# rubychen0611/image-analogies-python

Hardware: AMD Instinct MI355X
Metric: B' pixels/sec (brute-force match, 5-level pyramid) + MFMA util @1/2/4/8 GPU (higher is better)
Workload: dtype f16 rotated split (R16 MFMA screen: 3 principal components as f16 pairs, 52 as f16, f32 accumulate) + f64 (rotation, exact rescore, pyramids); 1 GPU; c4: A/A' 2048x2048 x B 1024x1024, 5-level, DB sharded, brute force; levels_cap=5, jobs_per_gpu=1, streams_per_gpu=1, jobs_per_launch=1, parallelism=single

## Files before the change

image-analogies-python_amd/csrc/ia_exact.h:

```cpp
#pragma once
#include "ia_imgwin.h"
#include "ia_split16.h"

#include <float.h>

namespace ia {

constexpr int TILE_H8 = DB16_GROUPS * 64;

__device__ __forceinline__ void best_update(double &bd, long long &bi, double d, long long i) {
    if (d < bd || (d == bd && i < bi)) { bd = d; bi = i; }
}

__device__ __forceinline__ void rescore_thresholds(float emin, float amax0, double nqq,
                                                   double &Tseg, double &Trow, bool &force_full) {
    constexpr double U32 = 5.9604644775390625e-08;
    const double A = (double)amax0;
    const double eps = 70.0 * U32 * (2.0 * A * sqrt(nqq) + A * A);
    const Split16Db sc = split16_db_scale(amax0);
    const int eq = split16_q_scale(nqq, sc.R);
    const int e2 = sc.ea + eq;
    const double em = ldexp((double)emin, -e2);
    const double eps16 = U32 * (300.0 * A * sqrt(nqq) + 50.0 * A * A);
    const double slack = 1e-12 * (fabs(em) + nqq + A * A);
    Tseg = ldexp(em + 2.0 * eps16 + slack, e2);
    Trow = ldexp(em + eps16 + eps + slack, sc.ea);
    force_full = eq + sc.R < -10;
}

__device__ __forceinline__ void load_row16(const half8 *__restrict__ db16, long r,
                                           half8 (&g0)[DB16_GROUPS], half8 (&g1)[DB16_GROUPS]) {
    const half8 *t = db16 + (r >> 5) * TILE_H8 + (r & 31);
#pragma unroll
    for (int g = 0; g < DB16_GROUPS; ++g) {
        g0[g] = t[g * 64];
        g1[g] = t[g * 64 + 32];
    }
}

__device__ __forceinline__ float rescreen16(const half8 (&g0)[DB16_GROUPS],
                                            const half8 (&g1)[DB16_GROUPS], const float *qf,
                                            float twoR) {
    float acc = 0.f;
#pragma unroll
    for (int k = 0; k < IA_DP; ++k) {
        _Float16 hi, lo;
        if (k < 24) { hi = g0[k >> 3][k & 7]; lo = g0[4 + (k >> 3)][k & 7]; }
        else if (k < 32) { hi = g0[3][k & 7]; lo = g1[3][k & 7]; }
        else { hi = g1[(k - 32) >> 3][k & 7]; lo = g1[4 + ((k - 32) >> 3)][k & 7]; }
        const float x = (float)hi + (float)lo;
        acc = fmaf(x, k < 55 ? qf[(k & 1) * 28 + (k >> 1)] : twoR, acc);
    }
    return acc;
}

__device__ __forceinline__ float win_x(const char *bf, const char *bc, int k) {
    const uint32_t v = *reinterpret_cast<const uint32_t *>(((k < 55 && win_coarse(k)) ? bc : bf) + win_off(k));
    return (float)__builtin_bit_cast(_Float16, (uint16_t)(v & 0xffffu)) +
           (float)__builtin_bit_cast(_Float16, (uint16_t)(v >> 16));
}
__device__ __forceinline__ void win_terms2(const char *r0, const char *r1, const float *qf, int k,
                                           float &a0, float &a1) {
    const uint32_t v0 = *reinterpret_cast<const uint32_t *>(r0);
    const uint32_t v1 = *reinterpret_cast<const uint32_t *>(r1);
    const float f = qf[(k & 1) * 28 + (k >> 1)];
    a0 = fmaf((float)__builtin_bit_cast(_Float16, (uint16_t)(v0 & 0xffffu)) +
              (float)__builtin_bit_cast(_Float16, (uint16_t)(v0 >> 16)), f, a0);
    a1 = fmaf((float)__builtin_bit_cast(_Float16, (uint16_t)(v1 & 0xffffu)) +
              (float)__builtin_bit_cast(_Float16, (uint16_t)(v1 >> 16)), f, a1);
}
__device__ __forceinline__ void rescreen_win2(const char *wb, int p, const float *qf, float twoR,
                                              float &e0, float &e1) {
    const char *bf0 = wb + 4 * p, *bc0 = wb + 4 * (p >> 1);
    const char *bf1 = bf0 + 256, *bc1 = bc0 + 128;
    float a0 = 0.f, a1 = 0.f;
    int k = 0;
#pragma unroll 1
    for (int r = 0; r < 3; ++r) {
        const int o = WB_FINE + r * WC_PC * 16 + 12;
#pragma unroll
        for (int c = 0; c < 3; ++c, ++k) win_terms2(bc0 + o + 4 * c, bc1 + o + 4 * c, qf, k, a0, a1);
    }
#pragma unroll 1
    for (int r = 0; r < 5; ++r) {
        const int o = r * WF_PC * 16 + 8;
#pragma unroll
        for (int c = 0; c < 5; ++c, ++k) win_terms2(bf0 + o + 4 * c, bf1 + o + 4 * c, qf, k, a0, a1);
    }
#pragma unroll 1
    for (int r = 3; r < 6; ++r) {
        const int o = WB_FINE + r * WC_PC * 16 + 12;
#pragma unroll
        for (int c = 0; c < 3; ++c, ++k) win_terms2(bc0 + o + 4 * c, bc1 + o + 4 * c, qf, k, a0, a1);
    }
#pragma unroll 1
    for (int r = 5; r < 8; ++r) {
        const int o = r * WF_PC * 16 + 8;
        const int nc = r < 7 ? 5 : 2;
#pragma unroll
        for (int c = 0; c < 5; ++c, ++k)
            if (c < nc) win_terms2(bf0 + o + 4 * c, bf1 + o + 4 * c, qf, k, a0, a1);
    }
    const uint32_t v0 = *reinterpret_cast<const uint32_t *>(bf0 + WB_FINE + WB_COARSE);
    const uint32_t v1 = *reinterpret_cast<const uint32_t *>(bf1 + WB_FINE + WB_COARSE);
    a0 = fmaf((float)__builtin_bit_cast(_Float16, (uint16_t)(v0 & 0xffffu)) +
              (float)__builtin_bit_cast(_Float16, (uint16_t)(v0 >> 16)), twoR, a0);
    a1 = fmaf((float)__builtin_bit_cast(_Float16, (uint16_t)(v1 & 0xffffu)) +
              (float)__builtin_bit_cast(_Float16, (uint16_t)(v1 >> 16)), twoR, a1);
    e0 = a0;
    e1 = a1;
}
static_assert(win_off(0) == WB_FINE + 12 && win_off(9) == 8 && win_off(34) == WB_FINE + 3 * WC_PC * 16 + 12 &&
                  win_off(43) == 5 * WF_PC * 16 + 8 && win_off(54) == 7 * WF_PC * 16 + 12 &&
                  win_off(55) == WB_FINE + WB_COARSE,
              "rescreen_win2 walks win_off's rows");

constexpr int WIN_PPL = (WIN_PIECES + 63) / 64;
typedef unsigned int piece_t __attribute__((ext_vector_type(4)));
__device__ __forceinline__ void win_load(const ImgDb &im, long lrow, int lane, piece_t (&pc)[WIN_PPL]) {
    const WinSrc ws = win_src(im, lrow);
#pragma unroll
    for (int j = 0; j < WIN_PPL; ++j) {
        const int i = lane + 64 * j;
        if (i < WIN_PIECES) pc[j] = *reinterpret_cast<const piece_t *>(win_piece(im, ws, i));
    }
}
constexpr int WIN_SLOT = WIN_PPL * 1024;
__device__ __forceinline__ void win_dma(const ImgDb &im, long lrow, int lane, char *wb) {
    asm volatile("" : "+v"(lane));
    const WinSrc ws = win_src(im, lrow);
#pragma unroll
    for (int j = 0; j < WIN_PPL; ++j) {
        const int i = lane + 64 * j;
        __builtin_amdgcn_global_load_lds((const void *)win_piece(im, ws, i < WIN_PIECES ? i : 0),
                                         (void *)(wb + j * 1024), 16, 0, 0);
    }
}
__device__ __forceinline__ void win_dma_wait() {
    asm volatile("s_waitcnt vmcnt(0)" ::: "memory");
    __builtin_amdgcn_wave_barrier();
}
__device__ __forceinline__ void win_store(char *wb, int lane, const piece_t (&pc)[WIN_PPL]) {
#pragma unroll
    for (int j = 0; j < WIN_PPL; ++j) {
        const int i = lane + 64 * j;
        if (i < WIN_PIECES) reinterpret_cast<piece_t *>(wb)[i] = pc[j];
    }
}
__device__ __forceinline__ void wave_lds_sync() {
    __builtin_amdgcn_fence(__ATOMIC_RELEASE, "wavefront");
    __builtin_amdgcn_wave_barrier();
    __builtin_amdgcn_fence(__ATOMIC_ACQUIRE, "wavefront");
}

constexpr int RESCORE_SEGCAP = 1024;
constexpr int RESCORE_REG = 8;
constexpr int RESCORE_RPT = 2;
constexpr int RESCORE_ROWCAP = 512;
static_assert(DB_SEG_MAX <= RESCORE_RPT * 256, "one re-screen step per segment");

__device__ __forceinline__ int vidx(int i) {
    asm volatile("" : "+v"(i));
    return i;
}

__device__ __forceinline__ void segmin_load(const float4 *sq4, long n4, float4 (&v)[RESCORE_REG]) {
    const int tid = threadIdx.x;
    const long lim = tid < 256 ? n4 : 0;
#pragma unroll
    for (int j = 0; j < RESCORE_REG; ++j) {
        const long i = tid + (long)j * 256;
        const float4 x = sq4[i < n4 ? i : 0];
        v[j] = i < lim ? x : make_float4(FLT_MAX, FLT_MAX, FLT_MAX, FLT_MAX);
    }
}
__device__ __forceinline__ float segmin_wave_min(const float4 *sq4, long n4, const float4 (&v)[RESCORE_REG]) {
    const int tid = threadIdx.x;
    const long lim = tid < 256 ? n4 : 0;
    float emin = FLT_MAX;
#pragma unroll
// ... 96 lines not shown
```

image-analogies-python_amd/csrc/ia_rot16.h:

```cpp
#pragma once
#include "ia_internal.h"
#include "ia_split16.h"

namespace ia {

#ifndef IA_R16_P
#define IA_R16_P 3
#endif
constexpr int R16_P = IA_R16_P;
constexpr int R16_NL = 2 * R16_P;
constexpr int R16_M0 = R16_NL + 1;
constexpr int R16_NH = R16_M0 + IA_D;
constexpr int R16_SLOTS = (R16_NH + 16) / 16 * 16;
constexpr int R16_MFMA = R16_SLOTS / 16;
constexpr int R16_TILE_H8 = R16_MFMA * 64;
constexpr int R16_ROW_B = R16_SLOTS * 2;
constexpr int R16_LD = 56;
constexpr int R16_ROT_FLOATS = 13 * 256;
constexpr int R16_ROT_B = R16_ROT_FLOATS * 4;

static inline size_t r16_askseg_off(long nrows) { return (size_t)db_rows_padded(nrows) * R16_ROW_B; }
static inline size_t r16_askc_off(long nrows) {
    return r16_askseg_off(nrows) + img_align((size_t)db_nsegs(nrows) * 4);
}
static inline const unsigned char *r16_askc(const void *dbr, long nrows) {
    return reinterpret_cast<const unsigned char *>(dbr) + r16_askc_off(nrows);
}
static_assert(R16_LD * R16_LD <= R16_ROT_FLOATS, "rotation buffer");

__host__ __device__ constexpr int r16_qpos(int s) {
    return (((s & 15) >> 3) * R16_MFMA + (s >> 4)) * 8 + (s & 7);
}
__host__ __device__ constexpr int r16_dgrp(int s, int j) { return (s >> 4) * 64 + ((s & 15) >> 3) * 32 + j; }

#ifndef IA_R16_SHAPE
#define IA_R16_SHAPE 16
#endif
constexpr bool R16_S16 = IA_R16_SHAPE == 16 && R16_MFMA == 4;
constexpr double R16_EPS_A2 = R16_S16 ? 90.0 : 60.0;
__device__ __forceinline__ double r16_eps(double A, double nqq, double Askip, double nsk) {
    constexpr double U32 = 5.9604644775390625e-08;
    return U32 * (360.0 * A * sqrt(nqq) + R16_EPS_A2 * A * A) + 0x1p-9 * 1.01 * Askip * sqrt(nsk);
}

__device__ __forceinline__ void r16_thresholds(float emin, float amax0, float askip, double nqq, double nsk,
                                               double &Tseg, bool &force_full) {
    const double A = (double)amax0;
    const Split16Db sc = split16_db_scale(amax0);
    const int eq = split16_q_scale(nqq, sc.R);
    const int e2 = sc.ea + eq;
    const double em = ldexp((double)emin, -e2);
    const double eps = r16_eps(A, nqq, (double)askip, nsk);
    const double slack = 1e-12 * (fabs(em) + nqq + A * A);
    Tseg = ldexp(em + 2.0 * eps + slack, e2);
    force_full = eq + sc.R < -10;
}

__device__ __forceinline__ double r16_kseg(float amax0, float askip, double nqq, double nsk) {
    const Split16Db sc = split16_db_scale(amax0);
    const int e2 = sc.ea + split16_q_scale(nqq, sc.R);
    return ldexp(0x1p-9 * 1.01 * sqrt(nsk) * (double)askip / 255.0, e2);
}
__device__ __forceinline__ void r16_tseg0(float umin, float amax0, double nqq, double &T0, bool &force_full) {
    const double A = (double)amax0;
    const Split16Db sc = split16_db_scale(amax0);
    const int eq = split16_q_scale(nqq, sc.R);
    const int e2 = sc.ea + eq;
    const double em = ldexp((double)umin, -e2);
    const double eps0 = r16_eps(A, nqq, 0.0, 0.0);
    const double slack = 1e-12 * (fabs(em) + nqq + A * A) + 0x1p-23 * fabs(em);
    T0 = ldexp(em + 2.0 * eps0 + slack, e2);
    force_full = eq + sc.R < -10;
}

__device__ __forceinline__ void r16_thresholds_rows(float emin, float amax0, float askip, double nqq, double nsk,
                                                    double &Tseg, double &Trow, bool &force_full) {
    constexpr double U32 = 5.9604644775390625e-08;
    const double A = (double)amax0;
    const Split16Db sc = split16_db_scale(amax0);
    const int eq = split16_q_scale(nqq, sc.R);
    const int e2 = sc.ea + eq;
    const double em = ldexp((double)emin, -e2);
    const double eps = r16_eps(A, nqq, (double)askip, nsk);
    const double epsq = 70.0 * U32 * (2.0 * A * sqrt(nqq) + A * A);
    const double slack = 1e-12 * (fabs(em) + nqq + A * A);
    Tseg = ldexp(em + 2.0 * eps + slack, e2);
    Trow = ldexp(em + eps + epsq + slack, sc.ea);
    force_full = eq + sc.R < -10;
}

__device__ __forceinline__ double r16_write_query(_Float16 *row, int lane, double d, double nq, float amax,
                                                  const float *rot, double *dq) {
    dq[lane] = lane < IA_D ? d : 0.0;
    asm volatile("s_waitcnt lgkmcnt(0)" ::: "memory");
    __builtin_amdgcn_wave_barrier();
    asm volatile("" ::: "memory");
    const int j = lane < IA_D ? lane : 0;
    double k0 = 0.0, k1 = 0.0, k2 = 0.0, k3 = 0.0;
#pragma unroll
    for (int k = 0; k < 52; k += 4) {
        k0 = fma((double)rot[(k + 0) * R16_LD + j], dq[k + 0], k0);
        k1 = fma((double)rot[(k + 1) * R16_LD + j], dq[k + 1], k1);
        k2 = fma((double)rot[(k + 2) * R16_LD + j], dq[k + 2], k2);
        k3 = fma((double)rot[(k + 3) * R16_LD + j], dq[k + 3], k3);
    }
    k0 = fma((double)rot[52 * R16_LD + j], dq[52], k0);
    k1 = fma((double)rot[53 * R16_LD + j], dq[53], k1);
    k2 = fma((double)rot[54 * R16_LD + j], dq[54], k2);
    const double kap = (k0 + k1) + (k2 + k3);
    double s2 = (lane >= R16_P && lane < IA_D) ? kap * kap : 0.0;
    for (int o = 32; o > 0; o >>= 1) s2 += __shfl_xor(s2, o);
    const Split16Db sc = split16_db_scale(amax);
    const int eq = split16_q_scale(nq, sc.R);
    if (lane < IA_D) {
        _Float16 h, l;
        split16d(ldexp(-2.0 * kap, eq), h, l);
        row[r16_qpos(R16_M0 + lane)] = h;
        if (lane < R16_P) {
            row[r16_qpos(2 * lane)] = h;
            row[r16_qpos(2 * lane + 1)] = l;
        }
    } else if (lane == IA_D) {
        const _Float16 n = (_Float16)ldexpf(1.f, eq + sc.R);
        row[r16_qpos(R16_NL)] = n;
        row[r16_qpos(R16_NH)] = n;
    } else if (lane > IA_D && R16_NH + (lane - IA_D) < R16_SLOTS) {
        row[r16_qpos(R16_NH + (lane - IA_D))] = (_Float16)0.f;
    }
    return s2;
}

}
```

image-analogies-python_amd/csrc/ia_xwave.hip:

```cpp
#include "ia_exact.h"
#include "ia_finish.h"
#include "ia_rot16.h"
#include "../../include/ia_diag.h"

#include <climits>

namespace ia {

__device__ __forceinline__ const double *feat_addr(const ImgPair &X, const ImgPair &Y, int r, int c,
                                                   int k, int &rr, int &cc) {
    const bool yk = k >= 34;
    const int kk = yk ? k - 34 : k;
    const bool coarse = kk < 9;
    const int t = coarse ? kk : kk - 9;
    const int xh = coarse ? X.hs : X.h, yh = coarse ? Y.hs : Y.h;
    const int xw = coarse ? X.ws : X.w, yw = coarse ? Y.ws : Y.w;
    const double *xb = coarse ? X.sm : X.lg, *yb = coarse ? Y.sm : Y.lg;
    const int h = yk ? yh : xh;
    const int w = yk ? yw : xw;
    const double *base = yk ? yb : xb;
    const int r0 = coarse ? (r >> 1) + t / 3 - 1 : r + t / 5 - 2;
    const int c0 = coarse ? (c >> 1) + t % 3 - 1 : c + t % 5 - 2;
    rr = symi2(r0, h);
    cc = symi2(c0, w);
// ... 611 lines not shown
__device__ __forceinline__ int clampi(int v, int lo, int hi) { return v < lo ? lo : (v > hi ? hi : v); }
__device__ __forceinline__ XsWin xs_window(const XArgs &a, long seg) {
    const DbSrc &src = a.src;
    XsWin w;
    w.g0 = a.row0 + seg_lrow(a.smap, seg, a.seg_rows, 0);
    int img;
    row_pos(w.g0, src.hw, src.A.w, img, w.y0, w.x0);
    w.nst = a.seg_rows >> 7;
    w.fa = src.A.lg;
    w.ca = src.A.sm;
    w.fp = src.Ap.lg + (long)img * src.hw;
    w.cp = src.Ap.sm + (long)img * src.hws;
    return w;
}
__device__ __forceinline__ int xs_fbase(const XsWin &w, int y, int x) { return (y - w.y0 + 2) * XS_FW + (x - w.x0 + 4); }
__device__ __forceinline__ int xs_cbase(const XsWin &w, int y, int x) {
    return ((y >> 1) - (w.y0 >> 1) + 1) * XS_CW + ((x >> 1) - (w.x0 >> 1) + 2);
}
__host__ __device__ constexpr bool xs_coarse(int k) { return k < 9 || (k >= 34 && k < 43); }
__host__ __device__ constexpr int xs_koff(int k) {
    return k < 9 ? XS_CA + (k / 3 - 1) * XS_CW + (k % 3 - 1)
         : k < 34 ? XS_FA + ((k - 9) / 5 - 2) * XS_FW + ((k - 9) % 5 - 2)
         : k < 43 ? XS_CP + ((k - 34) / 3 - 1) * XS_CW + ((k - 34) % 3 - 1)
         : XS_FP + ((k - 43) / 5 - 2) * XS_FW + ((k - 43) % 5 - 2);
}

struct XsFix {
    double v[XS_DMA][2];
    unsigned mask;
};
__device__ __forceinline__ const double *xs_piece(const XsWin &w, const ImgPair &A, int p, int &C, int &iw) {
    constexpr int FP = XS_FW / 2, CP = XS_CW / 2;
    const double *img = w.fa;
    int sr = 0;
    iw = A.w;
    C = 0;
    if (p < 8 * FP) {
        const int r = p / FP;
        sr = symi2(min(w.y0 - 2 + r, w.y0 + w.nst + 1), A.h);
        C = w.x0 - 4 + 2 * (p - r * FP);
    } else if ((p -= 8 * FP) < 6 * FP) {
        const int r = p / FP;
        img = w.fp;
        sr = symi2(min(w.y0 - 2 + r, w.y0 + w.nst - 1), A.h);
        C = w.x0 - 4 + 2 * (p - r * FP);
    } else if ((p -= 6 * FP) < 8 * CP) {
        const int r = p / CP;
        img = r < 4 ? w.ca : w.cp;
        iw = A.ws;
        sr = symi2(min((w.y0 >> 1) - 1 + (r & 3), ((w.y0 + w.nst - 1) >> 1) + 1), A.hs);
        C = (w.x0 >> 1) - 2 + 2 * (p - r * CP);
    }
    return img + (long)sr * iw;
}
__device__ __forceinline__ void xs_dma(const XsWin &w, const ImgPair &A, char *win, int dr, int lane, XsFix &fx) {
    asm volatile("" : "+v"(lane));
    fx.mask = 0;
#pragma unroll
    for (int j = 0; j < XS_DMA; ++j) {
        const int p = 192 * j + 64 * dr + lane;
        int C, iw;
        const double *row = xs_piece(w, A, p, C, iw);
        __builtin_amdgcn_global_load_lds((const void *)(row + clampi(C, 0, iw - 2)),
                                         (void *)(win + (192 * j + 64 * dr) * 16), 16, 0, 0);
        if (C < 0 || C + 1 >= iw) {
            fx.mask |= 1u << j;
            fx.v[j][0] = row[symi2(clampi(C, -2, iw + 1), iw)];
            fx.v[j][1] = row[symi2(clampi(C + 1, -2, iw + 1), iw)];
        }
    }
}
constexpr int XS_PRE = (XS_PIECES + 255) / 256;
struct XsPre {
    double v[XS_PRE][2];
};
__device__ __forceinline__ void xs_pre_load(const XsWin &w, const ImgPair &A, int tid, XsPre &pr) {
#pragma unroll
    for (int j = 0; j < XS_PRE; ++j) {
        const int p = 256 * j + tid;
        int C, iw;
        const double *row = xs_piece(w, A, p < XS_PIECES ? p : XS_PIECES - 1, C, iw);
        pr.v[j][0] = row[symi2(clampi(C, -2, iw + 1), iw)];
        pr.v[j][1] = row[symi2(clampi(C + 1, -2, iw + 1), iw)];
    }
}
__device__ __forceinline__ void xs_pre_store(const XsPre &pr, char *win, int tid) {
#pragma unroll
    for (int j = 0; j < XS_PRE; ++j) {
        const int p = 256 * j + tid;
        if (p < XS_PIECES) {
            double *d = reinterpret_cast<double *>(win + p * 16);
            d[0] = pr.v[j][0];
            d[1] = pr.v[j][1];
        }
    }
}
__device__ __forceinline__ void xs_fix(const XsFix &fx, char *win, int t) {
#pragma unroll
    for (int j = 0; j < XS_DMA; ++j)
        if (fx.mask & (1u << j)) {
            double *d = reinterpret_cast<double *>(win + (192 * j + t) * 16);
            d[0] = fx.v[j][0];
            d[1] = fx.v[j][1];
        }
}
template <int K0, int K1, typename F>
__device__ __forceinline__ void xs_for(F &&f) {
    if constexpr (K0 < K1) {
        f(std::integral_constant<int, K0>{});
        xs_for<K0 + 1, K1>(f);
    }
}
__device__ __forceinline__ void xs_dist2(const double *win, int f0, int c0, int f1, int c1, const double *qs,
                                         double &d0, double &d1) {
    Pw55 a, b;
    asm volatile("" : "+v"(f0), "+v"(c0), "+v"(f1), "+v"(c1));
    xs_for<0, IA_D>([&](auto kc) {
        constexpr int k = decltype(kc)::value;
        constexpr int o = xs_koff(k);
        const int b0 = xs_coarse(k) ? c0 : f0, b1 = xs_coarse(k) ? c1 : f1;
        const double q = qs[k];
        const double x0 = win[b0 + o] - q, x1 = win[b1 + o] - q;
        a.feed(k, x0 * x0);
        b.feed(k, x1 * x1);
    });
    d0 = a.res;
    d1 = b.res;
    asm volatile("" :: "v"(d0), "v"(d1));
}

__device__ __forceinline__ void xs_dist_pair(const double *win, int fb, int cb, const double *qs,
                                             double &d0, double &d1) {
    Pw55 a, b;
    asm volatile("" : "+v"(fb), "+v"(cb));
    xs_for<0, IA_D>([&](auto kc) {
        constexpr int k = decltype(kc)::value;
        constexpr int o = xs_koff(k);
        const double q = qs[k];
        if constexpr (xs_coarse(k)) {
            const double x = win[cb + o] - q;
            a.feed(k, x * x);
            b.feed(k, x * x);
        } else {
            const double x0 = win[fb + o] - q, x1 = win[fb + XS_FW + o] - q;
            a.feed(k, x0 * x0);
            b.feed(k, x1 * x1);
        }
    });
    d0 = a.res;
    d1 = b.res;
    asm volatile("" :: "v"(d0), "v"(d1));
}

__device__ __forceinline__ double pw55_lanes(double v) {
    const long long b = __double_as_longlong(v);
    const int lo = (int)b, hi = (int)(b >> 32);
    auto at = [&](int k) {
        return __longlong_as_double((long long)(((unsigned long long)(unsigned)__builtin_amdgcn_readlane(hi, k) << 32) |
                                                (unsigned)__builtin_amdgcn_readlane(lo, k)));
    };
    double r[8];
#pragma unroll
    for (int j = 0; j < 8; ++j) r[j] = at(j);
#pragma unroll
    for (int k = 8; k < 48; k += 8) {
#pragma unroll
        for (int j = 0; j < 8; ++j) r[j] += at(k + j);
    }
    double res = ((r[0] + r[1]) + (r[2] + r[3])) + ((r[4] + r[5]) + (r[6] + r[7]));
#pragma unroll
    for (int k = 48; k < IA_D; ++k) res += at(k);
    return res;
}

constexpr int XS_REG = 11;
template <int XR>
__device__ __forceinline__ void seg3_load(const float4 *sq4, long n4, int t3, float4 (&v)[XR]) {
#pragma unroll
    for (int j = 0; j < XR; ++j) {
        const long i = t3 + (long)j * 192;
        const float4 x = sq4[i < n4 ? i : 0];
        v[j] = i < n4 ? x : make_float4(FLT_MAX, FLT_MAX, FLT_MAX, FLT_MAX);
    }
}
template <int XR>
__device__ __forceinline__ float seg3_wave_min(const float4 *sq4, long n4, int t3, const float4 (&v)[XR]) {
    float emin = FLT_MAX;
#pragma unroll
    for (int j = 0; j < XR; ++j) emin = fminf(emin, fminf(fminf(v[j].x, v[j].y), fminf(v[j].z, v[j].w)));
    for (long i = t3 + (long)XR * 192; i < n4; i += 192) {
        const float4 x = sq4[i];
        emin = fminf(emin, fminf(fminf(x.x, x.y), fminf(x.z, x.w)));
    }
    for (int o = 32; o > 0; o >>= 1) emin = fminf(emin, __shfl_xor(emin, o));
    return emin;
}
template <int XR>
__device__ __forceinline__ void seg3_select(const float4 *sq4, long n4, int t3, const float4 (&v)[XR],
                                            double Tseg, int *slist, int *scount) {
    static_assert(XR * 4 <= 64, "one 64-bit mask");
    unsigned long long m = 0;
#pragma unroll
    for (int j = 0; j < XR; ++j) {
        m |= (unsigned long long)((double)v[j].x <= Tseg) << (4 * j);
        m |= (unsigned long long)((double)v[j].y <= Tseg) << (4 * j + 1);
        m |= (unsigned long long)((double)v[j].z <= Tseg) << (4 * j + 2);
        m |= (unsigned long long)((double)v[j].w <= Tseg) << (4 * j + 3);
    }
    if (m) {
        int pos = atomicAdd(scount, __builtin_popcountll(m));
        while (m) {
            const int b = __builtin_ctzll(m);
            m &= m - 1;
            if (pos < RESCORE_SEGCAP) slist[pos] = 4 * (t3 + (b >> 2) * 192) + (b & 3);
            ++pos;
        }
    }
    for (long i = t3 + (long)XR * 192; i < n4; i += 192) {
        const float4 x = sq4[i];
        unsigned mt = ((double)x.x <= Tseg ? 1u : 0u) | ((double)x.y <= Tseg ? 2u : 0u) |
                      ((double)x.z <= Tseg ? 4u : 0u) | ((double)x.w <= Tseg ? 8u : 0u);
        if (mt) {
            int pos = atomicAdd(scount, __builtin_popcount(mt));
            while (mt) {
                const int b = __builtin_ctz(mt);
                mt &= mt - 1;
                if (pos < RESCORE_SEGCAP) slist[pos] = (int)(4 * i + b);
                ++pos;
            }
        }
    }
}
template <int XR>
__device__ __forceinline__ void seg3_load_codes(const unsigned *ac4, long n4, int t3, unsigned (&cv)[XR]) {
#pragma unroll
    for (int j = 0; j < XR; ++j) {
        const long i = t3 + (long)j * 192;
        cv[j] = ac4[i < n4 ? i : 0];
    }
}
__device__ __forceinline__ float seg_uval(float m, unsigned c, int b, float Kf) {
    return fmaf(Kf, (float)((c >> (8 * b)) & 255u), m);
}
template <int XR>
__device__ __forceinline__ float seg3_wave_umin(const float4 *sq4, const unsigned *ac4, long n4, int t3,
                                                const float4 (&v)[XR], const unsigned (&cv)[XR], float Kf) {
    float u = FLT_MAX;
#pragma unroll
    for (int j = 0; j < XR; ++j)
        u = fminf(u, fminf(fminf(seg_uval(v[j].x, cv[j], 0, Kf), seg_uval(v[j].y, cv[j], 1, Kf)),
                           fminf(seg_uval(v[j].z, cv[j], 2, Kf), seg_uval(v[j].w, cv[j], 3, Kf))));
    for (long i = t3 + (long)XR * 192; i < n4; i += 192) {
        const float4 x = sq4[i];
        const unsigned c = ac4[i];
        u = fminf(u, fminf(fminf(seg_uval(x.x, c, 0, Kf), seg_uval(x.y, c, 1, Kf)),
                           fminf(seg_uval(x.z, c, 2, Kf), seg_uval(x.w, c, 3, Kf))));
    }
    for (int o = 32; o > 0; o >>= 1) u = fminf(u, __shfl_xor(u, o));
    return u;
}
__device__ __forceinline__ unsigned seg_sel4(const float4 &x, unsigned c, double T0, double K) {
    return ((double)x.x <= fma(K, (double)(c & 255u), T0) ? 1u : 0u) |
           ((double)x.y <= fma(K, (double)((c >> 8) & 255u), T0) ? 2u : 0u) |
           ((double)x.z <= fma(K, (double)((c >> 16) & 255u), T0) ? 4u : 0u) |
           ((double)x.w <= fma(K, (double)(c >> 24), T0) ? 8u : 0u);
}
template <int XR>
__device__ __forceinline__ void seg3_select_codes(const float4 *sq4, const unsigned *ac4, long n4, int t3,
                                                  const float4 (&v)[XR], const unsigned (&cv)[XR],
                                                  double T0, double K, int *slist, int *scount) {
    unsigned long long m = 0;
#pragma unroll
    for (int j = 0; j < XR; ++j) m |= (unsigned long long)seg_sel4(v[j], cv[j], T0, K) << (4 * j);
    if (m) {
        int pos = atomicAdd(scount, __builtin_popcountll(m));
        while (m) {
            const int b = __builtin_ctzll(m);
            m &= m - 1;
            if (pos < RESCORE_SEGCAP) slist[pos] = 4 * (t3 + (b >> 2) * 192) + (b & 3);
            ++pos;
        }
    }
    for (long i = t3 + (long)XR * 192; i < n4; i += 192) {
        unsigned mt = seg_sel4(sq4[i], ac4[i], T0, K);
        if (mt) {
            int pos = atomicAdd(scount, __builtin_popcount(mt));
            while (mt) {
                const int b = __builtin_ctz(mt);
                mt &= mt - 1;
                if (pos < RESCORE_SEGCAP) slist[pos] = (int)(4 * i + b);
                ++pos;
            }
        }
    }
}
__device__ __forceinline__ void sync3(unsigned *cnt, unsigned g, int lane) {
    asm volatile("s_waitcnt lgkmcnt(0)" ::: "memory");
    if (lane == 0) __hip_atomic_fetch_add(cnt, 1u, __ATOMIC_RELAXED, __HIP_MEMORY_SCOPE_WORKGROUP);
    while (__hip_atomic_load(cnt, __ATOMIC_RELAXED, __HIP_MEMORY_SCOPE_WORKGROUP) < 3u * g)
        __builtin_amdgcn_s_sleep(1);
    asm volatile("" ::: "memory");
}

#ifndef IA_XSTRIP_BOCC
#define IA_XSTRIP_BOCC 4
#endif
#ifndef IA_XSTRIP_BREG
#define IA_XSTRIP_BREG 2
#endif
template <bool BATCH, bool ROT>
__global__ __launch_bounds__(256, BATCH ? IA_XSTRIP_BOCC : 3) void k_xstrip(XArgs a0) {
    __shared__ __attribute__((aligned(16))) char sa_raw[BATCH ? sizeof(XArgs) : 16];
    XArgs &sa = *reinterpret_cast<XArgs *>(sa_raw);
    if constexpr (BATCH) {
        const unsigned long long *w0 = reinterpret_cast<const unsigned long long *>(&a0);
        unsigned long long *w1 = reinterpret_cast<unsigned long long *>(&sa);
        for (int w = threadIdx.x; w < (int)(sizeof(XArgs) / 8); w += 256) w1[w] = w0[w];
        __syncthreads();
        if (threadIdx.x == 0) xjob_apply(sa, a0.jobs[blockIdx.y], a0.f.t & 1);
        __syncthreads();
    }
    const XArgs &a = BATCH ? sa : a0;
    __shared__ __attribute__((aligned(16))) char win[XS_LDS_B];
    __shared__ double cxd[XW_NCOH * XS_CST];
    __shared__ double cval[XW_NCOH];
    __shared__ double qs[IA_DP], wts[IA_DP];
    __shared__ double cwt[2 * IA_DP];
    __shared__ int slist[RESCORE_SEGCAP];
    __shared__ int tk, scount, sfull;
    __shared__ unsigned bar3;
    __shared__ float redf[4];
    __shared__ double bds[4], bwd[4], bvl[4];
    __shared__ long long bis[4];
    __shared__ CohSel cs;
    __shared__ double csval;
    __shared__ long long ccix[XW_NCOH];
    __shared__ int cpos[XW_NCOH][3];
    __shared__ unsigned nxw[4][64];
    static_assert(R16_ROT_B + 64 * 8 <= XS_LDS_B, "the rotation fits the window buffer");
    float *const rotl = reinterpret_cast<float *>(win);
    double *const dq = reinterpret_cast<double *>(win + R16_ROT_B);

    const int tid = threadIdx.x, lane = tid & 63, wv = __builtin_amdgcn_readfirstlane(tid >> 6);
    const FinishArgs &f = a.f;
    const DbSrc &src = a.src;
    const int t = f.t, W = f.W;
    const unsigned long long t_start = __builtin_amdgcn_s_memrealtime();
    auto rot_dma = [&]() {
#pragma unroll
        for (int pc = 0; pc < R16_ROT_FLOATS / 256; ++pc)
            __builtin_amdgcn_global_load_lds((const void *)(a.rot.get() + pc * 256 + lane * 4),
                                             (void *)(rotl + pc * 256), 16, 0, 0);
    };
    if (tid == 0) {
        tk = (int)atomicAdd(&a.tickets[t & 1], 1u);
        bar3 = 0;
        scount = 0;
    }
    __syncthreads();
    const int i = tk;
    unsigned long long *trace =
        (a.trace && i < XW_TRACE_PX && t < XW_TRACE_T) ? a.trace + ((long)t * XW_TRACE_PX + i) * XW_TRACE_N : nullptr;
    auto wstamp = [&](int k) {
        if (trace && lane == 0) trace[k] = __builtin_amdgcn_s_memrealtime();
    };
    if (trace && tid == 0) trace[0] = t_start;
    xw_stamp(trace, 1);
    if (i == 0 && tid == 0) __hip_atomic_store(&a.tickets[(t + 1) & 1], 0u, __ATOMIC_RELAXED, __HIP_MEMORY_SCOPE_AGENT);
    const int y = f.y_lo + i, x = t - 3 * y;
    const bool cur = i < a.M;
    const bool nxt = y >= a.y_lo_n && y < a.y_lo_n + a.M_n;

    const float amx = a.amax[vidx(0)];
    int pdep = 0;
    if (wv == 0 && nxt) {
        int rr = 0, cc = 0;
        const double *p = feat_addr_v(a.B.sm, a.B.lg, a.Bp.sm, a.Bp.lg, a.B.h, a.B.w, a.B.hs, a.B.ws, y, x + 1,
                                      lane < IA_D ? lane : 0, rr, cc);
        pdep = lane < 43 || lane >= IA_D ? 0 : (rr == y && cc == x) ? 1 : (rr == y - 1 && cc == x + 3) ? 2 : 0;
        dma_f64(p, lane < IA_D && pdep == 0, nxw[0], nxw[1]);
        dma_f64(a.center + (lane < IA_D ? lane : 0), lane < IA_D, nxw[2], nxw[3]);
    }

    double own = 0.0;
    if (cur) {
        const int t3 = (wv == 0 ? 0 : wv - 1) * 64 + lane;
        const int ql = lane < IA_DP ? lane : 0;
        const double qsv = a.q64[(long)i * IA_DP + ql];
        const double wk0 = f.weights[lane < IA_D ? lane : 0];
        const double wk = lane < IA_D ? wk0 : 0.0;
        const double nqq = a.nq[vidx(i)];
        const double nsk = ROT ? a.q64[(long)i * IA_DP + IA_D] : 0.0;
        const float am = amx, ask = ROT ? a.amax[vidx(1)] : 0.f;
        const long n4 = a.nseg / 4;
        const float4 *sq4 = reinterpret_cast<const float4 *>(a.segmin + (long)i * a.nseg);
        constexpr int XR = BATCH ? IA_XSTRIP_BREG : XS_REG;
        float4 v[XR];
        unsigned sgc[XR];
        const unsigned *ac4 = ROT ? reinterpret_cast<const unsigned *>(a.askc.get()) : nullptr;
        if (wv != 1) {
            seg3_load(sq4, n4, t3, v);
            if constexpr (ROT) seg3_load_codes(ac4, n4, t3, sgc);
        }
        const int rr0 = y - 2 + lane / 5, rc0 = x - 2 + lane % 5;
        const bool cpos_ok = wv == 1 && lane < XW_NCOH && rr0 >= 0 && rc0 >= 0 && rc0 < W &&
                             (rr0 < y || rc0 < x);
        const long sidx = cpos_ok ? (long)rr0 * W + rc0 : 0;
        const int s_r = f.s[2 * sidx], s_c = f.s[2 * sidx + 1], s_i = f.im[sidx];
        asm volatile("" ::: "memory");
        double Kd = 0.0;
        if constexpr (ROT) Kd = r16_kseg(am, ask, nqq, nsk);
        if (wv != 1) {
            float ewv;
            if constexpr (ROT) {
                float Kf = (float)Kd;
                if ((double)Kf < Kd) Kf = nextafterf(Kf, INFINITY);
                ewv = seg3_wave_umin(sq4, ac4, n4, t3, v, sgc, Kf);
            } else {
                ewv = seg3_wave_min(sq4, n4, t3, v);
            }
            if (lane == 0) redf[wv] = ewv;
        }
        if (wv == 1) wstamp(14);
        double cv[XW_NCOH], cvl = 0.0;
        if (wv == 1) {
            int sr = s_r + y - rr0, sc = s_c + x - rc0;
            const bool ok = cpos_ok && sr >= 0 && sr < src.A.h && sc >= 0 && sc < src.A.w;
            sr = ok ? sr : 0;
            sc = ok ? sc : 0;
            const int si = ok ? s_i : 0;
            const long cix = ((long)src.A.h * si + sr) * src.A.w + sc;
            cvl = src.Ap.lg[cix];
            if (lane < XW_NCOH) {
                ccix[lane] = ok ? cix : -1;
                cpos[lane][0] = sr; cpos[lane][1] = sc; cpos[lane][2] = si;
            }
            const int k = lane < IA_D ? lane : 0;
            const bool yk = k >= 34;
            const int kk = yk ? k - 34 : k;
            const bool co = kk < 9;
            const int t = co ? kk : kk - 9;
            const int dy = co ? t / 3 - 1 : t / 5 - 2, dx = co ? t % 3 - 1 : t % 5 - 2;
            int Ah = src.A.h, Ahs = src.A.hs, Aw2 = src.A.w, Aws = src.A.ws;
            int hw = (int)src.hw, hws = (int)src.hws;
            const double *pAl = src.A.lg, *pAs = src.A.sm, *pPl = src.Ap.lg, *pPs = src.Ap.sm;
            asm volatile("" : "+v"(Ah), "+v"(Ahs), "+v"(Aw2), "+v"(Aws), "+v"(hw), "+v"(hws));
            asm volatile("" : "+v"(pAl), "+v"(pAs), "+v"(pPl), "+v"(pPs));
            const int ih = co ? Ahs : Ah, iw = co ? Aws : Aw2;
            const int sh = co ? 1 : 0;
            const int istr = yk ? (co ? hws : hw) : 0;
            const double *lb0 = yk ? (co ? pPs : pPl) : (co ? pAs : pAl);
            const int offk = dy * iw + dx;
#pragma unroll
            for (int c = 0; c < XW_NCOH; ++c) {
                const int r = __builtin_amdgcn_readlane(sr, c), cc = __builtin_amdgcn_readlane(sc, c);
                const int im = __builtin_amdgcn_readlane(si, c);
                const int rs = r >> sh, cs2 = cc >> sh;
                int off = rs * iw + cs2 + offk;
                if (!(r >= 2 && r + 2 < src.A.h && cc >= 2 && cc + 2 < src.A.w))
                    off = symi2(rs + dy, ih) * iw + symi2(cs2 + dx, iw);
                typedef const __attribute__((address_space(1))) double gdouble;
                cv[c] = *(gdouble *)(lb0 + ((long)im * istr + off));
            }
            wstamp(13);
        }
        if (wv == 1 && lane < IA_DP) {
            qs[lane] = qsv;
            wts[lane] = wk;
            cwt[lane] = 1.0;
            cwt[IA_DP + lane] = wk;
        }
        int ns = 0;
        bool full = false;
        if (wv != 1) {
            sync3(&bar3, 1, lane);
            const float emin = fminf(redf[0], fminf(redf[2], redf[3]));
            xw_stamp(trace, 2);
            double Tseg, Trow;
            bool force_full;
            if constexpr (ROT) {
                r16_tseg0(emin, am, nqq, Tseg, force_full);
                seg3_select_codes(sq4, ac4, n4, t3, v, sgc, Tseg, Kd, slist, &scount);
            } else {
                rescore_thresholds(emin, am, nqq, Tseg, Trow, force_full);
                seg3_select(sq4, n4, t3, v, Tseg, slist, &scount);
            }
            sync3(&bar3, 2, lane);
            xw_stamp(trace, 3);
            ns = scount;
            full = ns > RESCORE_SEGCAP || force_full;
            if (tid == 0) sfull = full ? 1 : 0;
            if (trace && tid == 0) trace[XW_TRACE_N - 1] = (unsigned long long)(full ? a.nseg : ns);
        }

        auto coherence = [&]() {
#pragma unroll
            for (int c = 0; c < XW_NCOH; ++c) cxd[c * XS_CST + lane] = cv[c];
            if (lane < XW_NCOH) cval[lane] = cvl;
            wave_lds_sync();
            const int c = (lane & 31) < XW_NCOH ? (lane & 31) : XW_NCOH - 1;
            const bool wl = lane >= 32;
            int co = c * XS_CST, qo = 0, wo = wl ? IA_DP : 0;
            asm volatile("" : "+v"(co), "+v"(qo), "+v"(wo));
            Pw55 pw;
#pragma unroll
            for (int k = 0; k < IA_D; ++k) {
                const double xx = (cxd[co + k] - qs[qo + k]) * cwt[wo + k];
                pw.feed(k, xx * xx);
                if (k % 11 == 10) asm volatile("" : "+v"(co), "+v"(qo), "+v"(wo) : "v"(xx));
            }
            const double r = sqrt(pw.res);
            asm volatile("" :: "v"(r));
            const bool valid = (lane & 31) < XW_NCOH && ccix[c] >= 0;
            double bd = valid && !wl ? r : INFINITY;
            long long bl = valid && !wl ? c : LLONG_MAX;
            const double cwd = r * r;
            for (int o = 32; o > 0; o >>= 1) {
                const double od = __shfl_xor(bd, o);
                const long long ol = __shfl_xor(bl, o);
                fin_best(bd, bl, od, ol);
            }
            const int wn = bl == LLONG_MAX ? 0 : (int)bl;
            const double wd = __shfl(cwd, 32 + wn);
            const double wval = cval[wn];
            wstamp(15);
            if (lane == 0) {
                cs = bl == LLONG_MAX ? CohSel{0, 0, 0, 0, 0, 0, 0, 0.0}
                                     : CohSel{ccix[wn], cpos[wn][0], cpos[wn][1], cpos[wn][2],
                                              y - 2 + wn / 5, x - 2 + wn % 5, 1, wd};
                csval = wval;
            }
        };

        double bd = INFINITY;
        long long bi = LLONG_MAX;
        const int Aw = src.A.w;
        XsWin w{};
        XsFix fx;
        const int dr = wv == 0 ? 0 : wv - 1;
        long nit = full ? a.nseg : ns;
        if (wv != 1 && nit > 0) {
            w = xs_window(a, full ? 0 : slist[0]);
            xs_dma(w, src.A, win, dr, lane, fx);
        }
        if (wv == 1) {
            coherence();
        } else if (nit > 0) {
            win_dma_wait();
            xs_fix(fx, win, 64 * dr + lane);
        }
        __syncthreads();
        if (wv == 1) {
            ns = scount;
            full = sfull != 0;
            nit = full ? a.nseg : ns;
            if (nit > 0) w = xs_window(a, full ? 0 : slist[0]);
        }
        const long nscan = nit;
        XsPre pre;
        XsWin wn{};
        for (long si = 0; si < nit; ++si) {
            if (si > 0) {
                __syncthreads();
                xs_pre_store(pre, win, tid);
                w = wn;
                __syncthreads();
            }
            if (si + 1 < nit) {
                wn = xs_window(a, full ? si + 1 : slist[si + 1]);
                xs_pre_load(wn, src.A, tid, pre);
            }
            if (si == 0) {
                xw_stamp(trace, 4);
                if (wv == 0) wstamp(11);
            }
            const double *wdb = reinterpret_cast<const double *>(win);
            if (w.nst == 4) {
                const int px = w.x0 + (tid & 127), py = w.y0 + 2 * (tid >> 7);
                double d0, d1;
                xs_dist_pair(wdb, xs_fbase(w, py, px), xs_cbase(w, py, px), qs, d0, d1);
                const long g = w.g0 + (long)(2 * (tid >> 7)) * Aw + (tid & 127);
                fin_best(bd, bi, d0, g);
                fin_best(bd, bi, d1, g + Aw);
            } else {
                const int k0 = tid & (a.seg_rows - 1), k1 = (tid + 256) & (a.seg_rows - 1);
                const int y0 = w.y0 + (k0 >> 7), x0 = w.x0 + (k0 & 127);
                const int y1 = w.y0 + (k1 >> 7), x1 = w.x0 + (k1 & 127);
                double d0, d1;
                xs_dist2(wdb, xs_fbase(w, y0, x0), xs_cbase(w, y0, x0), xs_fbase(w, y1, x1), xs_cbase(w, y1, x1),
                         qs, d0, d1);
                if (tid < a.seg_rows) fin_best(bd, bi, d0, w.g0 + (long)(k0 >> 7) * Aw + (k0 & 127));
                if (tid + 256 < a.seg_rows) fin_best(bd, bi, d1, w.g0 + (long)(k1 >> 7) * Aw + (k1 & 127));
            }
            if (si == 0 && wv == 0) wstamp(12);
        }
        for (int o = 32; o > 0; o >>= 1) {
            const double od = __shfl_xor(bd, o);
            const long long oi = __shfl_xor(bi, o);
            fin_best(bd, bi, od, oi);
        }
        XRec wb{bd, bi, 0.0, 0.0};
        if (bi != LLONG_MAX) {
            const long rel = bi - w.g0;
            const long ry = rel >= 0 ? rel / Aw : -1, rx = rel - ry * Aw;
            double sq = 0.0;
            if (rel >= 0 && ry < w.nst && rx < 128) {
                const int py = w.y0 + (int)ry, px = w.x0 + (int)rx;
                const int fb = xs_fbase(w, py, px), cb = xs_cbase(w, py, px);
                const double *wdb = reinterpret_cast<const double *>(win);
                if (lane < IA_D) {
                    const double xw = (wdb[(xs_coarse(lane) ? cb : fb) + xs_koff(lane)] - qs[lane]) * wts[lane];
                    sq = xw * xw;
                }
                wb.val = wdb[XS_FP + fb];
            } else {
                ImgPair ap;
                int r, c;
                src.locate(bi, ap, r, c);
                int rr, cc;
                const double *fp = feat_addr(src.A, ap, r, c, lane < IA_D ? lane : 0, rr, cc);
                if (lane < IA_D) {
                    const double xw = (*fp - qs[lane]) * wts[lane];
                    sq = xw * xw;
                }
                wb.val = src.Ap.lg[bi];
            }
            const double sw = sqrt(pw55_lanes(sq));
            wb.wd = sw * sw;
        }
        if (lane == 0) { bds[wv] = wb.d; bis[wv] = wb.i; bwd[wv] = wb.wd; bvl[wv] = wb.val; }
        __syncthreads();
        xw_stamp(trace, 5);
        if (wv != 0) return;
        if constexpr (ROT) {
            if (nxt) rot_dma();
        }
        XRec lb{INFINITY, LLONG_MAX, 0.0, 0.0};
#pragma unroll
        for (int k = 0; k < 4; ++k) xrec_take(lb, XRec{bds[k], bis[k], bwd[k], bvl[k]});
        xw_stamp(trace, 6);
        own = xw_finish(a, i, y, x, lane, lb, cs, csval, (unsigned int)(nscan * a.seg_rows), ns, full, trace);
    }
    xw_stamp(trace, 8);
    if (wv != 0 || !nxt) return;
    if constexpr (ROT) {
        if (!cur) rot_dma();
    }
    xw_next_query(a, i, y, x, lane, pdep, own, amx, nxw, trace, ROT ? rotl : nullptr, ROT ? dq : nullptr);
}

}

extern "C" int ia_fused_resources(int rot, int *lds, int *vgprs) {
    IA_ARG(lds && vgprs, "ia_fused_resources: bad args");
    hipFuncAttributes at{};
    if (rot) IA_HIP(hipFuncGetAttributes(&at, reinterpret_cast<const void *>(&ia::k_xstrip<false, true>)));
    else IA_HIP(hipFuncGetAttributes(&at, reinterpret_cast<const void *>(&ia::k_xstrip<false, false>)));
    *lds = (int)at.sharedSizeBytes;
    *vgprs = at.numRegs;
    return IA_OK;
}

namespace ia {

int xwave_attributes(int form, bool rot, hipFuncAttributes *at) {
    const void *f = form == XW_STRIP ? (rot ? reinterpret_cast<const void *>(&k_xstrip<false, true>)
                                            : reinterpret_cast<const void *>(&k_xstrip<false, false>))
                    : form == XW_IMG ? reinterpret_cast<const void *>(&k_xwave<true, false>)
                                     : reinterpret_cast<const void *>(&k_xwave<false, false>);
    IA_HIP(hipFuncGetAttributes(at, f));
    return IA_OK;
}

int launch_xwave(const XArgs &a, int nblocks, int form, hipStream_t st, int njobs) {
    if (nblocks <= 0) return IA_OK;
    IA_ARG(njobs >= 1 && njobs <= IA_BATCH_MAX && (njobs == 1 || a.jobs), "launch_xwave: bad batch");
    IA_ARG(form != XW_STRIP || (a.smap.W > 0 && xstrip_applies(a.src) && a.seg_rows >= 128 && a.seg_rows <= 512),
           "launch_xwave: the strip form needs a strip-order image-form level");
    const dim3 grid((unsigned)nblocks, (unsigned)njobs);
    const bool b = njobs > 1;
    if (form == XW_STRIP) {
        if (a.rot) {
            if (b) k_xstrip<true, true><<<grid, 256, 0, st>>>(a);
            else k_xstrip<false, true><<<grid, 256, 0, st>>>(a);
        } else {
            if (b) k_xstrip<true, false><<<grid, 256, 0, st>>>(a);
            else k_xstrip<false, false><<<grid, 256, 0, st>>>(a);
        }
    } else if (form == XW_IMG) {
        if (b) k_xwave<true, true><<<grid, 256, 0, st>>>(a);
        else k_xwave<true, false><<<grid, 256, 0, st>>>(a);
    } else {
        if (b) k_xwave<false, true><<<grid, 256, 0, st>>>(a);
        else k_xwave<false, false><<<grid, 256, 0, st>>>(a);
    }
    IA_LAUNCH_CHECK("k_xwave");
    return IA_OK;
}

}
```

Before: 1.861 million B' pixels/s.

## Sort candidate segments by lower bound and prune exact rescore early

During segment selection, each candidate's screen minimum and skip code are now stashed in a small shared-memory area. When 2 to 64 segments survive, the wave ranks them by lower bound with readlane and ds_permute, rescores them in ascending order, and skips any segment whose bound exceeds the current exact best after a DPP wave-min reduction. The goal is to avoid exact f64 distance evaluation and window DMA for segments that cannot win. In exchange it adds per-iteration reductions and an extra block sync. It also shrinks the segment capacity to make room for the stash, so more queries may fall back to a full scan.

```diff
diff --git a/image-analogies-python_amd/csrc/ia_exact.h b/image-analogies-python_amd/csrc/ia_exact.h
--- a/image-analogies-python_amd/csrc/ia_exact.h
+++ b/image-analogies-python_amd/csrc/ia_exact.h
@@ -26,6 +26,14 @@
     Tseg = ldexp(em + 2.0 * eps16 + slack, e2);
     Trow = ldexp(em + eps16 + eps + slack, sc.ea);
     force_full = eq + sc.R < -10;
+}
+
+__device__ __forceinline__ void rescore_prune0(float amax0, double nqq, double &P0, int &e2) {
+    constexpr double U32 = 5.9604644775390625e-08;
+    const double A = (double)amax0;
+    const Split16Db sc = split16_db_scale(amax0);
+    e2 = sc.ea + split16_q_scale(nqq, sc.R);
+    P0 = U32 * (300.0 * A * sqrt(nqq) + 50.0 * A * A) - nqq + 2e-12 * (nqq + A * A);
 }
 
 __device__ __forceinline__ void load_row16(const half8 *__restrict__ db16, long r,
diff --git a/image-analogies-python_amd/csrc/ia_rot16.h b/image-analogies-python_amd/csrc/ia_rot16.h
--- a/image-analogies-python_amd/csrc/ia_rot16.h
+++ b/image-analogies-python_amd/csrc/ia_rot16.h
@@ -73,6 +73,13 @@
     force_full = eq + sc.R < -10;
 }
 
+__device__ __forceinline__ void r16_prune0(float amax0, double nqq, double &P0, int &e2) {
+    const double A = (double)amax0;
+    const Split16Db sc = split16_db_scale(amax0);
+    e2 = sc.ea + split16_q_scale(nqq, sc.R);
+    P0 = r16_eps(A, nqq, 0.0, 0.0) - nqq + 2e-12 * (nqq + A * A);
+}
+
 __device__ __forceinline__ void r16_thresholds_rows(float emin, float amax0, float askip, double nqq, double nsk,
                                                     double &Tseg, double &Trow, bool &force_full) {
     constexpr double U32 = 5.9604644775390625e-08;
diff --git a/image-analogies-python_amd/csrc/ia_xwave.hip b/image-analogies-python_amd/csrc/ia_xwave.hip
--- a/image-analogies-python_amd/csrc/ia_xwave.hip
+++ b/image-analogies-python_amd/csrc/ia_xwave.hip
@@ -787,6 +787,25 @@
     asm volatile("" :: "v"(d0), "v"(d1));
 }
 
+__device__ __forceinline__ double wave_min63(double v) {
+#define IA_DPP_MIN64(CTRL, ROWS)                                                                          \
+    {                                                                                                     \
+        const long long b = __double_as_longlong(v);                                                      \
+        const unsigned lo = (unsigned)__builtin_amdgcn_update_dpp((int)b, (int)b, CTRL, ROWS, 0xf, false); \
+        const unsigned hi =                                                                               \
+            (unsigned)__builtin_amdgcn_update_dpp((int)(b >> 32), (int)(b >> 32), CTRL, ROWS, 0xf, false); \
+        v = fmin(v, __longlong_as_double((long long)(((unsigned long long)hi << 32) | lo)));              \
+    }
+    IA_DPP_MIN64(0x111, 0xf);
+    IA_DPP_MIN64(0x112, 0xf);
+    IA_DPP_MIN64(0x114, 0xf);
+    IA_DPP_MIN64(0x118, 0xf);
+    IA_DPP_MIN64(0x142, 0xa);
+    IA_DPP_MIN64(0x143, 0xc);
+#undef IA_DPP_MIN64
+    return v;
+}
+
 __device__ __forceinline__ double pw55_lanes(double v) {
     const long long b = __double_as_longlong(v);
     const int lo = (int)b, hi = (int)(b >> 32);
@@ -830,9 +849,41 @@
     for (int o = 32; o > 0; o >>= 1) emin = fminf(emin, __shfl_xor(emin, o));
     return emin;
 }
+constexpr int XS_SORT = 64;
+constexpr int XS_STASH = XS_SORT + XS_SORT / 4 + 8;
+constexpr int XS_SEGCAP = RESCORE_SEGCAP - XS_STASH;
+static_assert((XS_SEGCAP + XS_SORT + XS_SORT / 4) % 2 == 0, "bdw is 8-byte aligned");
+__device__ __forceinline__ void seg_put(int &pos, int seg, float m, unsigned c, int *slist, float *skey,
+                                        unsigned char *scode) {
+    if (pos < XS_SEGCAP) slist[pos] = seg;
+    if (pos < XS_SORT) {
+        skey[pos] = m;
+        scode[pos] = (unsigned char)c;
+    }
+    ++pos;
+}
+__device__ __forceinline__ float f4_at(const float4 &x, int e) {
+    return e == 0 ? x.x : e == 1 ? x.y : e == 2 ? x.z : x.w;
+}
+template <int XR>
+__device__ __forceinline__ void seg_pick(const float4 (&v)[XR], const unsigned *cv, int b, float &m, unsigned &c) {
+    float4 x = v[0];
+    unsigned cc = cv ? cv[0] : 0u;
+#pragma unroll
+    for (int j = 1; j < XR; ++j) {
+        const bool h = (b >> 2) == j;
+        x.x = h ? v[j].x : x.x;
+        x.y = h ? v[j].y : x.y;
+        x.z = h ? v[j].z : x.z;
+        x.w = h ? v[j].w : x.w;
+        if (cv) cc = h ? cv[j] : cc;
+    }
+    m = f4_at(x, b & 3);
+    c = (cc >> (8 * (b & 3))) & 255u;
+}
 template <int XR>
 __device__ __forceinline__ void seg3_select(const float4 *sq4, long n4, int t3, const float4 (&v)[XR],
-                                            double Tseg, int *slist, int *scount) {
+                                            double Tseg, int *slist, int *scount, float *skey, unsigned char *scode) {
     static_assert(XR * 4 <= 64, "one 64-bit mask");
     unsigned long long m = 0;
 #pragma unroll
@@ -847,8 +898,10 @@
         while (m) {
             const int b = __builtin_ctzll(m);
             m &= m - 1;
-            if (pos < RESCORE_SEGCAP) slist[pos] = 4 * (t3 + (b >> 2) * 192) + (b & 3);
-            ++pos;
+            float mv;
+            unsigned c;
+            seg_pick(v, nullptr, b, mv, c);
+            seg_put(pos, 4 * (t3 + (b >> 2) * 192) + (b & 3), mv, 0u, slist, skey, scode);
         }
     }
     for (long i = t3 + (long)XR * 192; i < n4; i += 192) {
@@ -860,8 +913,7 @@
             while (mt) {
                 const int b = __builtin_ctz(mt);
                 mt &= mt - 1;
-                if (pos < RESCORE_SEGCAP) slist[pos] = (int)(4 * i + b);
-                ++pos;
+                seg_put(pos, (int)(4 * i + b), f4_at(x, b), 0u, slist, skey, scode);
             }
         }
     }
@@ -903,7 +955,8 @@
 template <int XR>
 __device__ __forceinline__ void seg3_select_codes(const float4 *sq4, const unsigned *ac4, long n4, int t3,
                                                   const float4 (&v)[XR], const unsigned (&cv)[XR],
-                                                  double T0, double K, int *slist, int *scount) {
+                                                  double T0, double K, int *slist, int *scount, float *skey,
+                                                  unsigned char *scode) {
     unsigned long long m = 0;
 #pragma unroll
     for (int j = 0; j < XR; ++j) m |= (unsigned long long)seg_sel4(v[j], cv[j], T0, K) << (4 * j);
@@ -912,19 +965,22 @@
         while (m) {
             const int b = __builtin_ctzll(m);
             m &= m - 1;
-            if (pos < RESCORE_SEGCAP) slist[pos] = 4 * (t3 + (b >> 2) * 192) + (b & 3);
-            ++pos;
+            float mv;
+            unsigned c;
+            seg_pick(v, cv, b, mv, c);
+            seg_put(pos, 4 * (t3 + (b >> 2) * 192) + (b & 3), mv, c, slist, skey, scode);
         }
     }
     for (long i = t3 + (long)XR * 192; i < n4; i += 192) {
-        unsigned mt = seg_sel4(sq4[i], ac4[i], T0, K);
+        const float4 x = sq4[i];
+        const unsigned cc = ac4[i];
+        unsigned mt = seg_sel4(x, cc, T0, K);
         if (mt) {
             int pos = atomicAdd(scount, __builtin_popcount(mt));
             while (mt) {
                 const int b = __builtin_ctz(mt);
                 mt &= mt - 1;
-                if (pos < RESCORE_SEGCAP) slist[pos] = (int)(4 * i + b);
-                ++pos;
+                seg_put(pos, (int)(4 * i + b), f4_at(x, b), (cc >> (8 * b)) & 255u, slist, skey, scode);
             }
         }
     }
@@ -961,7 +1017,10 @@
     __shared__ double cval[XW_NCOH];
     __shared__ double qs[IA_DP], wts[IA_DP];
     __shared__ double cwt[2 * IA_DP];
-    __shared__ int slist[RESCORE_SEGCAP];
+    __shared__ __attribute__((aligned(8))) int slist[RESCORE_SEGCAP];
+    float *const skey = reinterpret_cast<float *>(slist + XS_SEGCAP);
+    unsigned char *const scode = reinterpret_cast<unsigned char *>(slist + XS_SEGCAP + XS_SORT);
+    double *const bdw = reinterpret_cast<double *>(slist + XS_SEGCAP + XS_SORT + XS_SORT / 4);
     __shared__ int tk, scount, sfull;
     __shared__ unsigned bar3;
     __shared__ float redf[4];
@@ -1044,12 +1103,15 @@
         const int s_r = f.s[2 * sidx], s_c = f.s[2 * sidx + 1], s_i = f.im[sidx];
         asm volatile("" ::: "memory");
         double Kd = 0.0;
-        if constexpr (ROT) Kd = r16_kseg(am, ask, nqq, nsk);
+        float Kf = 0.f;
+        if constexpr (ROT) {
+            Kd = r16_kseg(am, ask, nqq, nsk);
+            Kf = (float)Kd;
+            if ((double)Kf < Kd) Kf = nextafterf(Kf, INFINITY);
+        }
         if (wv != 1) {
             float ewv;
             if constexpr (ROT) {
-                float Kf = (float)Kd;
-                if ((double)Kf < Kd) Kf = nextafterf(Kf, INFINITY);
                 ewv = seg3_wave_umin(sq4, ac4, n4, t3, v, sgc, Kf);
             } else {
                 ewv = seg3_wave_min(sq4, n4, t3, v);
@@ -1115,15 +1177,15 @@
             bool force_full;
             if constexpr (ROT) {
                 r16_tseg0(emin, am, nqq, Tseg, force_full);
-                seg3_select_codes(sq4, ac4, n4, t3, v, sgc, Tseg, Kd, slist, &scount);
+                seg3_select_codes(sq4, ac4, n4, t3, v, sgc, Tseg, Kd, slist, &scount, skey, scode);
             } else {
                 rescore_thresholds(emin, am, nqq, Tseg, Trow, force_full);
-                seg3_select(sq4, n4, t3, v, Tseg, slist, &scount);
+                seg3_select(sq4, n4, t3, v, Tseg, slist, &scount, skey, scode);
             }
             sync3(&bar3, 2, lane);
             xw_stamp(trace, 3);
-            ns = scount;
-            full = ns > RESCORE_SEGCAP || force_full;
+            ns = __builtin_amdgcn_readfirstlane(scount);
+            full = ns > XS_SEGCAP || force_full;
             if (tid == 0) sfull = full ? 1 : 0;
             if (trace && tid == 0) trace[XW_TRACE_N - 1] = (unsigned long long)(full ? a.nseg : ns);
         }
@@ -1173,10 +1235,48 @@
         XsWin w{};
         XsFix fx;
         const int dr = wv == 0 ? 0 : wv - 1;
-        long nit = full ? a.nseg : ns;
+        int nit = full ? (int)a.nseg : ns;
+        int sseg = 0;
+        double slb = 0.0;
+        bool srt = false;
+        int o_sg = 0, o_rank = 0;
+        float o_m = 0.f;
+        unsigned o_c = 0;
+        auto order1 = [&]() -> long {
+            srt = !full && ns >= 2 && ns <= XS_SORT;
+            if (!srt) return full ? 0 : slist[0];
+            const int k = lane < ns ? lane : 0;
+            o_sg = slist[k];
+            o_m = skey[k];
+            o_c = ROT ? scode[k] : 0u;
+            const float u = ROT ? fmaf(Kf, (float)o_c, o_m) : o_m;
+            o_rank = 0;
+            for (int j = 0; j < ns; ++j) {
+                const float uj = __int_as_float(__builtin_amdgcn_readlane(__float_as_int(u), j));
+                o_rank += (uj < u || (uj == u && j < lane)) ? 1 : 0;
+            }
+            if (lane >= ns) o_rank = lane;
+            return __builtin_amdgcn_readlane(o_sg, __builtin_ctzll(__ballot(o_rank == 0)));
+        };
+        auto order2 = [&]() {
+            if (!srt) return;
+            double P0;
+            int pe2;
+            if constexpr (ROT) r16_prune0(am, nqq, P0, pe2);
+            else rescore_prune0(am, nqq, P0, pe2);
+            const long long lb = __double_as_longlong(ldexp(fma(-Kd, (double)o_c, (double)o_m), -pe2) - P0);
+            sseg = __builtin_amdgcn_ds_permute(4 * o_rank, o_sg);
+            const unsigned lo = (unsigned)__builtin_amdgcn_ds_permute(4 * o_rank, (int)lb);
+            const unsigned hi = (unsigned)__builtin_amdgcn_ds_permute(4 * o_rank, (int)(lb >> 32));
+            slb = __longlong_as_double((long long)(((unsigned long long)hi << 32) | lo));
+        };
+        auto seg_at = [&](int k) -> long {
+            return full ? k : srt ? (long)__builtin_amdgcn_readlane(sseg, k) : (long)slist[k];
+        };
         if (wv != 1 && nit > 0) {
-            w = xs_window(a, full ? 0 : slist[0]);
+            w = xs_window(a, order1());
             xs_dma(w, src.A, win, dr, lane, fx);
+            order2();
         }
         if (wv == 1) {
             coherence();
@@ -1186,23 +1286,31 @@
         }
         __syncthreads();
         if (wv == 1) {
-            ns = scount;
+            ns = __builtin_amdgcn_readfirstlane(scount);
             full = sfull != 0;
-            nit = full ? a.nseg : ns;
-            if (nit > 0) w = xs_window(a, full ? 0 : slist[0]);
-        }
-        const long nscan = nit;
+            nit = full ? (int)a.nseg : ns;
+            if (nit > 0) {
+                w = xs_window(a, order1());
+                order2();
+            }
+        }
+        double bmax = INFINITY;
+        auto live = [&](int k) -> bool {
+            if (!srt) return true;
+            const long long lb = __double_as_longlong(slb);
+            const unsigned lo = (unsigned)__builtin_amdgcn_readlane((int)lb, k);
+            const unsigned hi = (unsigned)__builtin_amdgcn_readlane((int)(lb >> 32), k);
+            const bool skip = __longlong_as_double((long long)(((unsigned long long)hi << 32) | lo)) > bmax;
+            return __builtin_amdgcn_readfirstlane(skip ? 1 : 0) == 0;
+        };
         XsPre pre;
         XsWin wn{};
-        for (long si = 0; si < nit; ++si) {
-            if (si > 0) {
-                __syncthreads();
-                xs_pre_store(pre, win, tid);
-                w = wn;
-                __syncthreads();
-            }
-            if (si + 1 < nit) {
-                wn = xs_window(a, full ? si + 1 : slist[si + 1]);
+        int nscan = 0;
+        for (int si = 0; si < nit;) {
+            int nx = si + 1;
+            while (nx < nit && !live(nx)) ++nx;
+            if (nx < nit) {
+                wn = xs_window(a, seg_at(nx));
                 xs_pre_load(wn, src.A, tid, pre);
             }
             if (si == 0) {
@@ -1228,6 +1336,27 @@
                 if (tid + 256 < a.seg_rows) fin_best(bd, bi, d1, w.g0 + (long)(k1 >> 7) * Aw + (k1 & 127));
             }
             if (si == 0 && wv == 0) wstamp(12);
+            ++nscan;
+            if (nx >= nit) break;
+            if (srt) {
+                const double wm = wave_min63(bd);
+                if (lane == 63) bdw[wv] = wm;
+            }
+            __syncthreads();
+            if (srt) {
+                const double best = fmin(fmin(bdw[0], bdw[1]), fmin(bdw[2], bdw[3]));
+                bmax = fma(best, 2e-12, best);
+                if (!live(nx)) {
+                    do ++nx; while (nx < nit && !live(nx));
+                    if (nx >= nit) break;
+                    wn = xs_window(a, seg_at(nx));
+                    xs_pre_load(wn, src.A, tid, pre);
+                }
+            }
+            xs_pre_store(pre, win, tid);
+            w = wn;
+            __syncthreads();
+            si = nx;
         }
         for (int o = 32; o > 0; o >>= 1) {
             const double od = __shfl_xor(bd, o);
@@ -1274,7 +1403,7 @@
 #pragma unroll
         for (int k = 0; k < 4; ++k) xrec_take(lb, XRec{bds[k], bis[k], bwd[k], bvl[k]});
         xw_stamp(trace, 6);
-        own = xw_finish(a, i, y, x, lane, lb, cs, csval, (unsigned int)(nscan * a.seg_rows), ns, full, trace);
+        own = xw_finish(a, i, y, x, lane, lb, cs, csval, (unsigned int)nscan * (unsigned int)a.seg_rows, ns, full, trace);
     }
     xw_stamp(trace, 8);
     if (wv != 0 || !nxt) return;
```

Result: no change. 1.866 million B' pixels/s (median of 6 runs) (+0.3%).
